# citibeth/icebin

Measured on AMD Instinct MI355X. Metric: regridded cells/sec (AvI, g5, 64 fields/GPU), higher is better.
Workload: dtype f64

## Files before the change

icebin_amd/_capi.py:

```python
import ctypes as C
import os

import numpy as np

_HERE = os.path.dirname(os.path.abspath(__file__))
LIB_PATH = os.environ.get("ICEBIN_HIP_LIB") or os.path.join(_HERE, "lib", "libicebin_hip.so")

IBH_OK, IBH_EINVAL, IBH_ENODEVICE, IBH_EHIP, IBH_ERANGE, IBH_ENOTIMPL, IBH_ENOKEY = 0, -1, -2, -3, -4, -5, -6


class IcebinHipError(RuntimeError):

    def __init__(self, code, msg):
        super().__init__(msg)
        self.code = code


class RegridderDesc(C.Structure):
    _fields_ = [
        ("nX", C.c_int64), ("ex_indices", C.c_void_p), ("ex_area", C.c_void_p), ("nI", C.c_int64),
        ("nA", C.c_int64), ("nA_dense", C.c_int32), ("A_to_sparse", C.c_void_p),
        ("A_native_area", C.c_void_p), ("A_proj_area", C.c_void_p),
        ("nhc", C.c_int32), ("hcdefs", C.c_void_p), ("hc_stride_A", C.c_int64), ("hc_stride_HC", C.c_int64),
        ("interp_style", C.c_int32), ("I_centroid_xy", C.c_void_p),
# ... 51 lines not shown
                                              C.c_void_p, C.POINTER(C.c_void_p)]),
    "ibh_regrid_matrices_matrix_batch": (C.c_int, [C.c_void_p, C.c_int32, C.c_void_p, C.c_void_p, C.c_void_p, C.c_void_p,
                                                  C.c_void_p, C.c_void_p, C.c_void_p]),
    "ibh_regrid_matrices_matrix": (C.c_int, [C.c_void_p, C.c_char_p, C.POINTER(C.c_void_p)]),
    "ibh_weighted_from_coo": (C.c_int, [C.c_int32, C.c_int32, C.c_int64, C.c_void_p, C.c_void_p, C.c_void_p,
                                       C.c_void_p, C.c_void_p, C.c_int, C.c_int, C.POINTER(C.c_void_p)]),
    "ibh_weighted_from_csr": (C.c_int, [C.c_int32, C.c_int32, C.c_void_p, C.c_void_p, C.c_void_p, C.c_void_p,
                                       C.c_void_p, C.c_int, C.c_int, C.POINTER(C.c_void_p)]),
    "ibh_e1ve0_compute": (C.c_int, [C.c_int32, C.c_void_p, C.c_void_p, C.c_int64, C.POINTER(C.c_void_p)]),
    "ibh_weighted_make_I2vX": (C.c_int, [C.c_void_p, C.c_void_p, C.c_double, C.c_void_p, C.c_int64, C.c_void_p,
                                        C.POINTER(C.c_void_p)]),
    "ibh_weighted_destroy": (C.c_int, [C.c_void_p]),
    "ibh_weighted_shape": (C.c_int, [C.c_void_p, C.POINTER(C.c_int32), C.POINTER(C.c_int32), C.POINTER(C.c_int64)]),
    "ibh_weighted_flags": (C.c_int, [C.c_void_p, C.POINTER(C.c_int), C.POINTER(C.c_int)]),
    "ibh_weighted_dim": (C.c_int, [C.c_void_p, C.c_int, C.POINTER(C.c_int64), C.POINTER(C.c_int32)]),
    "ibh_weighted_dim_to_sparse": (C.c_int, [C.c_void_p, C.c_int, C.c_void_p]),
    "ibh_weighted_get_wM": (C.c_int, [C.c_void_p, C.c_void_p]),
    "ibh_weighted_get_Mw": (C.c_int, [C.c_void_p, C.c_void_p]),
    "ibh_weighted_get_coo": (C.c_int, [C.c_void_p, C.c_void_p, C.c_void_p, C.c_void_p]),
    "ibh_weighted_get_csr": (C.c_int, [C.c_void_p, C.c_void_p, C.c_void_p, C.c_void_p]),
    "ibh_weighted_apply_host": (C.c_int, [C.c_void_p, C.c_void_p, C.c_int32, C.c_int64, C.c_void_p, C.c_int64,
                                         C.c_double, C.c_int]),
    "ibh_weighted_apply_device": (C.c_int, [C.c_void_p, C.c_void_p, C.c_int32, C.c_int64, C.c_void_p, C.c_int64,
                                           C.c_double, C.c_int, C.c_void_p]),
    "ibh_weighted_apply_many_device": (C.c_int, [C.c_void_p, C.c_int32, C.c_void_p, C.c_int32, C.c_int64, C.c_void_p,
                                                C.c_int64, C.c_double, C.c_int, C.c_void_p]),
    "ibh_weighted_matvec_device": (C.c_int, [C.c_void_p, C.c_void_p, C.c_int32, C.c_int64, C.c_void_p, C.c_int64, C.c_int,
                                            C.c_void_p]),
    "ibh_coo_matvec": (C.c_int, [C.c_void_p, C.c_void_p, C.c_int, C.c_int64, C.c_int64, C.c_int64, C.c_void_p, C.c_void_p,
                                C.c_void_p]),
    "ibh_weighted_reserve": (C.c_int, [C.c_void_p, C.c_int32]),
    "ibh_weighted_prepare": (C.c_int, [C.c_void_p, C.c_int32, C.c_int32]),
    "ibh_weighted_pair_prepare": (C.c_int, [C.c_void_p, C.c_void_p, C.c_int32]),
    "ibh_weighted_apply_chain_device": (C.c_int, [C.c_void_p, C.c_void_p, C.c_void_p, C.c_void_p, C.c_int32, C.c_int64, C.c_void_p, C.c_int64,
                                               C.c_void_p, C.c_int64, C.c_void_p, C.c_int64, C.c_double, C.c_void_p]),
    "ibh_weighted_apply_pair_device": (C.c_int, [C.c_void_p, C.c_void_p, C.c_void_p, C.c_int32, C.c_int64, C.c_void_p, C.c_int64,
                                               C.c_void_p, C.c_int64, C.c_double, C.c_void_p]),
    "ibh_comm_unique_id": (C.c_int, [C.c_char_p]),
    "ibh_comm_create": (C.c_int, [C.c_int, C.c_int, C.c_char_p, C.POINTER(C.c_void_p)]),
    "ibh_comm_create_custom": (C.c_int, [C.c_int, C.c_int, C.c_void_p, C.c_void_p, C.POINTER(C.c_void_p)]),
    "ibh_comm_destroy": (C.c_int, [C.c_void_p]),
    "ibh_comm_info": (C.c_int, [C.c_void_p, C.POINTER(C.c_int), C.POINTER(C.c_int)]),
    "ibh_comm_wait": (C.c_int, [C.c_void_p, C.c_void_p]),
    "ibh_comm_set_custom_gatherv": (C.c_int, [C.c_void_p, C.c_void_p]),
    "ibh_comm_set_stream": (C.c_int, [C.c_void_p, C.c_void_p]),
    "ibh_comm_set_option": (C.c_int, [C.c_void_p, C.c_char_p, C.c_int]),
    "ibh_regrid_matrices_matrix_d_sharded": (C.c_int, [C.c_void_p, C.c_void_p, C.c_char_p, C.c_void_p, C.c_void_p, C.c_int, C.c_int,
                                                       C.POINTER(C.c_void_p)]),
    "ibh_weighted_apply_many_sharded_device": (C.c_int, [C.c_void_p, C.c_void_p, C.c_int32, C.c_void_p, C.c_int32, C.c_int64, C.c_void_p,
                                                        C.c_int64, C.c_double, C.c_void_p]),
    "ibh_weighted_apply_sharded_device": (C.c_int, [C.c_void_p, C.c_void_p, C.c_void_p, C.c_int32, C.c_int64, C.c_void_p, C.c_int64,
                                                   C.c_double, C.c_int32, C.c_void_p]),
    "ibh_regrid_matrices_matrix_d_sharded_sigma": (C.c_int, [C.c_void_p, C.c_void_p, C.c_char_p, C.c_void_p, C.c_void_p, C.c_int, C.c_int,
                                                             C.c_void_p, C.POINTER(C.c_void_p)]),
    "ibh_weighted_apply_many_sharded_conserve_device": (C.c_int, [C.c_void_p, C.c_void_p, C.c_int32, C.c_void_p, C.c_int32, C.c_int64,
                                                                 C.c_void_p, C.c_int64, C.c_double, C.c_int, C.c_void_p]),
    "ibh_weighted_apply_sharded_conserve_device": (C.c_int, [C.c_void_p, C.c_void_p, C.c_void_p, C.c_int32, C.c_int64, C.c_void_p,
                                                            C.c_int64, C.c_double, C.c_int, C.c_int32, C.c_void_p]),
    "ibh_weighted_apply_transformed_device": (C.c_int, [C.c_void_p, C.c_void_p, C.c_int32, C.c_int64, C.c_void_p,
                                                       C.c_void_p, C.c_int32, C.c_void_p, C.c_int64, C.c_double,
                                                       C.c_void_p]),
    "ibh_weighted_apply_weight_host": (C.c_int, [C.c_void_p, C.c_int, C.c_void_p, C.c_int32, C.c_int64, C.c_void_p]),
    "ibh_weighted_device_view_get": (C.c_int, [C.c_void_p, C.POINTER(DeviceView)]),
    "ibh_weighted_set_kernel": (C.c_int, [C.c_void_p, C.c_char_p]),
    "ibh_weighted_last_kernel": (C.c_int, [C.c_void_p, C.c_char_p, C.c_int]),
    "ibh_event_create": (C.c_int, [C.POINTER(C.c_void_p)]),
# ... 95 lines not shown
```

icebin_amd/csrc/capi.hip:

```cpp
#include <algorithm>
#include <cmath>
#include <map>
#include <memory>
#include <mutex>

#include "assemble.h"
#include "common.h"
#include "prims.h"

namespace ibh {

static thread_local std::string g_last_error;
void set_last_error(const char *msg) { g_last_error = msg ? msg : ""; }
void fail(int code, const char *fmt, ...) {
    char buf[1024];
    va_list ap;
    va_start(ap, fmt);
    vsnprintf(buf, sizeof(buf), fmt, ap);
    va_end(ap);
    throw Error(code, buf);
}

namespace {
struct Pool {
// ... 521 lines not shown
        if (val) w->val.download(val, (size_t)w->nnz);
    });
}

int ibh_weighted_apply_device(const ibh_weighted *w, const double *dA, int32_t nvar, int64_t lda, double *dB,
                              int64_t ldb, double fill, int force_conservation, void *stream) {
    return guarded([&] {
        check_weighted_device(w);
        IBH_CHECK(nvar >= 0 && (nvar == 0 || (dA && dB)), "bad arguments");
        spmm_launch(w, dA, nvar, lda, dB, ldb, fill, force_conservation, static_cast<hipStream_t>(stream));
    });
}
int ibh_weighted_apply_many_device(const ibh_weighted *w, int32_t nbatch, const double *const *dA, int32_t nvar,
                                   int64_t lda, double *const *dB, int64_t ldb, double fill, int force_conservation,
                                   void *stream) {
    return guarded([&] {
        check_weighted_device(w);
        IBH_CHECK(nbatch >= 0 && nvar >= 0 && (nbatch == 0 || nvar == 0 || (dA && dB)), "bad arguments");
        spmm_launch_many(w, nbatch, dA, nvar, lda, dB, ldb, fill, force_conservation, static_cast<hipStream_t>(stream));
    });
}
int ibh_weighted_reserve(const ibh_weighted *w, int32_t nvar) {
    return guarded([&] {
        check_weighted_device(w);
        IBH_CHECK(nvar >= 0, "bad arguments");
        weighted_reserve(w, nvar);
    });
}
int ibh_weighted_prepare(const ibh_weighted *w, int32_t nvar, int32_t nbatch) {
    return guarded([&] {
        check_weighted_device(w);
        IBH_CHECK(nvar >= 0 && nbatch >= 0, "bad arguments");
        weighted_prepare(w, nvar, nbatch);
    });
}
int ibh_weighted_pair_prepare(const ibh_weighted *first, const ibh_weighted *second, int32_t nvar) {
    return guarded([&] {
        check_weighted_device(first);
        check_weighted_device(second);
        IBH_CHECK(nvar >= 0, "bad arguments");
        weighted_pair_prepare(first, second, nvar);
    });
}
int ibh_weighted_apply_pair_device(const ibh_weighted *first, const ibh_weighted *second, const double *dA, int32_t nvar, int64_t lda,
                                   double *dB1, int64_t ldb1, double *dB2, int64_t ldb2, double fill, void *stream) {
    return guarded([&] {
        check_weighted_device(first);
        check_weighted_device(second);
        IBH_CHECK(nvar >= 0 && (nvar == 0 || (dA && dB1 && dB2)), "bad arguments");
        spmm_launch_pair(first, second, dA, nvar, lda, dB1, ldb1, dB2, ldb2, fill, static_cast<hipStream_t>(stream));
    });
}
int ibh_weighted_apply_chain_device(const ibh_weighted *first, const ibh_weighted *second, const ibh_weighted *third, const double *dA, int32_t nvar,
                                    int64_t lda, double *dB1, int64_t ldb1, double *dB2, int64_t ldb2, double *dB3, int64_t ldb3, double fill,
                                    void *stream) {
    return guarded([&] {
        check_weighted_device(first);
        check_weighted_device(second);
        check_weighted_device(third);
        IBH_CHECK(nvar >= 0 && (nvar == 0 || (dA && dB1 && dB2 && dB3)), "bad arguments");
        IBH_CHECK(nvar == 0 || ldb3 >= third->nrow, "chain apply: leading dimension %ld smaller than %d rows", (long)ldb3, third->nrow);
        spmm_launch_chain(first, second, third, dA, nvar, lda, dB1, ldb1, dB2, ldb2, dB3, ldb3, fill, static_cast<hipStream_t>(stream));
    });
}
int ibh_weighted_apply_host(const ibh_weighted *w, const double *A_b, int32_t nvar, int64_t lda, double *B_b,
                            int64_t ldb, double fill, int force_conservation) {
// ... 275 lines not shown
```

icebin_amd/csrc/common.h:

```cpp
#pragma once
#include <atomic>
#include <mutex>
#include <hip/hip_runtime.h>

#include <cstdarg>
#include <cstdint>
#include <cstdio>
#include <cstring>
#include <new>
#include <stdexcept>
#include <string>
#include <unordered_map>
#include <vector>

#include "../../include/icebin_hip.h"

namespace ibh {

struct Error : std::exception {
    int code;
    std::string msg;
    Error(int c, std::string m) : code(c), msg(std::move(m)) {}
    const char *what() const noexcept override { return msg.c_str(); }
};
// ... 192 lines not shown
    mutable int64_t band_n = 0;
    mutable ibh::DevBuf<int32_t> band_ptr, band_col, band_rb1;
    mutable ibh::DevBuf<double> band_v0, band_v1;
    int band_eligible = 0;
    int64_t band_sA = 0, band_sHC = 0;
    mutable int band_tried = 0;
    mutable int64_t napply = 0;
    mutable ibh::DevBuf<double> band_part;
    mutable int sweep_tried = 0;
    mutable int32_t sweep_ntask = 0, sweep_nblk = 0, sweep_nprow = 0, sweep_nslot = 0;
    mutable int32_t sweep_tb = 0, sweep_nitems = 0, sweep_ident = 0;
    mutable ibh::DevBuf<int32_t> sweep_task_p0, sweep_task_ns, sweep_col;
    mutable ibh::DevBuf<uint32_t> sweep_meta;
    mutable ibh::DevBuf<double> sweep_v0, sweep_v1;
    mutable ibh::DevBuf<int32_t> sweep_comb_ptr, sweep_comb_p;
    mutable ibh::DevBuf<double> sweep_part;
    mutable int grp_tried = 0;
    mutable const ibh_weighted *pair_second = nullptr;
    mutable uint64_t pair_uid = 0;
    mutable ibh::DevBuf<double> pair_w;
    mutable ibh::DevBuf<uint32_t> pair_mask;
    mutable ibh::DevBuf<int32_t> pair_row;
    mutable int32_t grp_n = 0, grp_nslot = 0, grp_nitems = 0;
    mutable ibh::DevBuf<int32_t> grp_ptr, grp_ns, grp_slotrow, grp_col;
    mutable ibh::DevBuf<uint32_t> grp_meta;
    mutable ibh::DevBuf<double> grp_v0, grp_v1;
    mutable int32_t gt_ntile = 0, gt_seg = 0;
    mutable ibh::DevBuf<int32_t> gt_ptr, gt_col;
    mutable ibh::DevBuf<uint16_t> gt_ek, gt_eptr;
    mutable ibh::DevBuf<double> gt_ev;
    mutable bool have_rowsum1 = false;
    mutable ibh::DevBuf<int32_t> rowperm;
    mutable bool have_rowperm = false;
    ~ibh_weighted() {
        for (int k = 0; k < 2; ++k)
            if (owns[k]) delete dims[k];
    }
};

struct ibh_exgrid {
    int64_t nX = 0;
    ibh::DevBuf<int32_t> indices;
    ibh::DevBuf<double> overlaps;
};

namespace ibh {
int comm_world(const ibh_comm *c);
int comm_rank(const ibh_comm *c);
void comm_exchange_blocks(ibh_comm *c, double *base, int64_t count, int64_t stride, hipStream_t st);
void comm_gatherv(ibh_comm *c, int n, void *const *bases, const int64_t *const *offs, hipStream_t st);
void spmm_launch(const ibh_weighted *w, const double *dA, int nvar, int64_t lda, double *dB, int64_t ldb,
                 double fill, int force_conservation, hipStream_t stream);
void spmm_launch_many(const ibh_weighted *w, int nbatch, const double *const *dA, int nvar, int64_t lda,
                      double *const *dB, int64_t ldb, double fill, int force_conservation, hipStream_t stream);
void weighted_reserve(const ibh_weighted *w, int nvar);
void weighted_prepare(const ibh_weighted *w, int nvar, int nbatch);
void weighted_pair_prepare(const ibh_weighted *first, const ibh_weighted *second, int nvar);
void spmm_launch_pair(const ibh_weighted *first, const ibh_weighted *second, const double *dA, int nvar, int64_t lda, double *dB1,
                      int64_t ldb1, double *dB2, int64_t ldb2, double fill, hipStream_t stream);
void spmm_launch_chain(const ibh_weighted *first, const ibh_weighted *second, const ibh_weighted *third, const double *dA, int nvar, int64_t lda,
                       double *dB1, int64_t ldb1, double *dB2, int64_t ldb2, double *dB3, int64_t ldb3, double fill, hipStream_t stream);
void build_bands_from_csr(const ibh_weighted *w, hipStream_t st);
bool build_sweep_from_csr(const ibh_weighted *w, hipStream_t st);
bool build_groups_from_csr(const ibh_weighted *w, hipStream_t st);
void matvec_legacy_launch(const ibh_weighted *w, const double *dx, int nvar, int64_t ldx, double *dy, int64_t ldy,
                          int ignore_nan, hipStream_t stream);
void spmm_transformed_launch(const ibh_weighted *w, const double *dA, int nvar_in, int64_t lda, const double *T,
                              const double *b, int nvar_out, double *dB, int64_t ldb, double fill, hipStream_t stream);
void weight_dot_launch(const double *dw, int n, const double *dA, int nvar, int64_t lda, double *dout, double *part,
                       hipStream_t stream);
size_t weight_dot_scratch(int n, int nvar);
void set_launch_events(hipEvent_t start, hipEvent_t stop);
int get_tuning(const char *key, int dflt);
void set_tuning(const char *key, int value);
}
```

icebin_amd/csrc/spmm.hip:

```cpp
#include "common.h"
#include "sweep_kernel.inl"
#include <hip/hip_ext.h>
#include <mutex>

namespace ibh {

namespace {
struct Tuning {
    std::mutex mu;
    std::unordered_map<std::string, int> map;
};
Tuning &tuning() { static Tuning *t = new Tuning; return *t; }
}
static thread_local const ibh_weighted *tl_handle = nullptr;
struct HandleScope {
    const ibh_weighted *prev;
    explicit HandleScope(const ibh_weighted *w) : prev(tl_handle) { tl_handle = w; }
    ~HandleScope() { tl_handle = prev; }
};
int get_tuning(const char *key, int dflt) {
    if (tl_handle && !tl_handle->opts.empty()) {
        auto it = tl_handle->opts.find(key);
        if (it != tl_handle->opts.end()) return it->second;
    }
// ... 304 lines not shown
        const int n = min(SEG, end - seg);
        int cc[ST];
        double vv[ST];
#pragma unroll
        for (int i = 0; i < ST; ++i) {
            const int k = min((int)threadIdx.x + i * T, n - 1);
            cc[i] = colind[seg + k];
            vv[i] = vals[seg + k];
        }
        if (seg != beg) __syncthreads();
#pragma unroll
        for (int i = 0; i < ST; ++i) {
            const int k = threadIdx.x + i * T;
            if (k < n) { s_col[k] = cc[i]; s_val[k] = vv[i]; }
        }
        __syncthreads();
        double x[U];
#pragma unroll
        for (int u = 0; u < U; ++u) {
            const int k = lane + 64 * u;
            x[u] = xload(rs, s_col[k < n ? k : n - 1] << 3);
        }
        __builtin_amdgcn_sched_barrier(0);
#pragma unroll
        for (int u = 0; u < U; ++u) {
            const int k = lane + 64 * u;
            const bool ok = k < n;
            const double v = s_val[ok ? k : n - 1];
            acc = ok ? fma(v, x[u], acc) : acc;
        }
    }
    acc = wave_sum(acc);
    if (lane == 0 && fw < nf) Y[(long)fw * ldy + r] = wM[r] == 0.0 ? fill : acc;
}

struct GroupView {
    const int *ptr, *ns, *slotrow, *col;
    const unsigned *meta;
    const double *v0, *v1;
    int ngrp, nslot;
};
constexpr unsigned RG_HAS0 = 1u << 16, RG_HAS1 = 1u << 17;
struct PairView {
    const double *w;
    const unsigned *mask;
    const int *row;
    const double *wM2;
    double *Y2;
    long ldy2;
};
template <int NW, int U, int TW, bool PAIR = false>
__global__ __launch_bounds__(NW * 64) void spmm_rowgroup_kernel(const GroupView gv, const BatchPtrs bp, long ldx, int ncol, long ldy, int nf,
                                                               int nfc, int xcd_mode, const double *__restrict__ wM, double fill,
                                                               const PairView pv = PairView{})
{
    constexpr int T = NW * 64, SEG = U * 64, ST = SEG / T;
    static_assert(SEG % T == 0, "segment is a multiple of the workgroup");
    extern __shared__ double rg_lds[];
    double *s_v0 = rg_lds, *s_v1 = rg_lds + SEG;
    int *s_col = reinterpret_cast<int *>(rg_lds + 2 * SEG);
    unsigned *s_meta = reinterpret_cast<unsigned *>(s_col + SEG);
    double *s_tab = rg_lds + 3 * SEG;
    int g, fc;
    if (!block_to_task(blockIdx.x, gv.ngrp, nfc, xcd_mode, g, fc)) return;
    const int lane = threadIdx.x & 63;
    const int wave = __builtin_amdgcn_readfirstlane(threadIdx.x >> 6);
// ... 606 lines not shown
        hipExtLaunchKernelGGL((spmm_rowblock_kernel<FPW, WK, U, NW>), grid, dim3(NW * 64), 0, stream, ev0, ev1, 0,  \
                              w->rowptr.p, w->colind.p, w->val.p, bp, nbatch, qi, lda, w->ncol, ldb, w->nrow, nvar, nfc, xcd_mode, w->wM.p, fill, \
                              (const double *)nullptr, (double *)nullptr, (const int *)rowperm, 0l);     \
    } while (0)
    if (unroll == 1) IBH_RB(1);
    else if (unroll == 2) IBH_RB(2);
    else if (unroll == 8) IBH_RB(8);
    else if (unroll > 8 && FPW == 1 && WK == 1) {
        if constexpr (FPW == 1 && WK == 1 && NW == 8) {
            if (unroll <= 12) IBH_RB(12); else if (unroll <= 14) IBH_RB(14); else IBH_RB(16);
        } else IBH_RB(8);
    }
    else IBH_RB(4);
#undef IBH_RB
    IBH_HIP(hipGetLastError());
}

template <int NW, int U>
static void launch_rowone(const ibh_weighted *w, const double *X, double *Y, int nvar, long lda, long ldb, double fill, hipStream_t stream)
{
    const int nfc = ceil_div(nvar, NW);
    int xcd_mode;
    const long nb = rowblock_grid(w->nrow, nfc, xcd_mode);
    IBH_CHECK(nb < (1l << 31), "spmm grid too large (%ld blocks)", nb);
    IBH_CHECK((long)w->ncol * 8 < (1l << 31), "ncol too large for 32-bit buffer offsets");
    hipEvent_t ev0 = g_ev_start, ev1 = g_ev_stop;
    g_ev_start = g_ev_stop = nullptr;
    snprintf(w->last_sig, sizeof(w->last_sig), "spmm_rowone_kernel<%d, %d>", NW, U);
    hipExtLaunchKernelGGL((spmm_rowone_kernel<NW, U>), dim3((unsigned)nb), dim3(NW * 64), 0, stream, ev0, ev1, 0, w->rowptr.p, w->colind.p,
                          w->val.p, X, Y, lda, w->ncol, ldb, w->nrow, nvar, nfc, xcd_mode, w->wM.p, fill);
    IBH_HIP(hipGetLastError());
}

template <int NW, int U, int TW>
static void launch_rowgroup(const ibh_weighted *w, const BatchPtrs &bp, int nbatch, int nvar, long lda, long ldb, double fill, hipStream_t stream,
                            const PairView *pair = nullptr)
{
    const int nfc = ceil_div(nvar, NW);
    int xcd_mode;
    const long nb = rowblock_grid(w->grp_n, nfc, xcd_mode);
    IBH_CHECK(nb < (1l << 31), "spmm grid too large (%ld blocks)", nb);
    IBH_CHECK((long)w->ncol * 8 < (1l << 31), "ncol too large for 32-bit buffer offsets");
    GroupView gv{w->grp_ptr.p, w->grp_ns.p, w->grp_slotrow.p, w->grp_col.p, w->grp_meta.p, w->grp_v0.p, w->grp_v1.p, w->grp_n, w->grp_nslot};
    const size_t lds = (size_t)(3 * U * 64 + NW * w->grp_nslot * TW) * sizeof(double);
    hipEvent_t ev0 = g_ev_start, ev1 = g_ev_stop;
    g_ev_start = g_ev_stop = nullptr;
    if (lds > 64 * 1024) {
        static std::mutex mu;
        static bool raised[64] = {};
        std::lock_guard<std::mutex> lk(mu);
        if (!raised[w->device & 63]) {
            IBH_HIP(hipFuncSetAttribute(reinterpret_cast<const void *>(spmm_rowgroup_kernel<NW, U, TW>), hipFuncAttributeMaxDynamicSharedMemorySize, 160 * 1024));
            raised[w->device & 63] = true;
        }
    }
    snprintf(w->last_sig, sizeof(w->last_sig), "spmm_rowgroup_kernel<%d, %d, %d, %s>", NW, U, TW, pair ? "true" : "false");
    if (pair) {
        IBH_CHECK(lds <= 64 * 1024 && nbatch == 1, "fused pair apply: %zu bytes of LDS / %d batches not supported", lds, nbatch);
        hipExtLaunchKernelGGL((spmm_rowgroup_kernel<NW, U, TW, true>), dim3((unsigned)nb, 1u), dim3(NW * 64), lds, stream, ev0, ev1, 0, gv, bp,
                              lda, w->ncol, ldb, nvar, nfc, xcd_mode, w->wM.p, fill, *pair);
    } else
        hipExtLaunchKernelGGL((spmm_rowgroup_kernel<NW, U, TW>), dim3((unsigned)nb, (unsigned)nbatch), dim3(NW * 64), lds, stream, ev0, ev1, 0, gv, bp,
                              lda, w->ncol, ldb, nvar, nfc, xcd_mode, w->wM.p, fill, PairView{});
    IBH_HIP(hipGetLastError());
}

// ... 273 lines not shown
        try { build_bands_from_csr(w, stream); }
        catch (const Error &) { (void)hipGetLastError(); drop_bands(w); }
    }
}

static void size_scratch(const ibh_weighted *w, int nvar, int nbatch) {
    if (w->band_n > 0) grow_scratch(w->band_part, band_part_count(w, nvar, nbatch), nullptr, "band");
    if (w->sweep_ntask > 0) grow_scratch(w->sweep_part, sweep_part_count(w, nvar, nbatch), nullptr, "column-sweep");
    if (pick_kernel(w, nvar, nbatch) == KERNEL_SHORTROW || pick_kernel(w, nvar, 1) == KERNEL_SHORTROW || w->kernel_override == KERNEL_AUTO) {
        for (int nb : {1, nbatch}) {
            const ShortrowPlan p = shortrow_plan(w, nvar, nb);
            const int qmax = std::max(1, get_tuning("shortrow_many", w->nrow >= (1 << 19) ? 1 : IBH_MAX_BATCH));
            if (p.use_xt && (pick_kernel(w, nvar, nb) == KERNEL_SHORTROW || w->kernel_override == KERNEL_SHORTROW))
                grow_scratch(w->xt, (size_t)w->ncol * (size_t)p.ldt * (size_t)std::min(qmax, nb), nullptr, "transposed-input");
        }
    }
    grow_scratch(w->consv, 2 * (size_t)nvar + weight_dot_scratch(std::max(w->nrow, w->ncol), nvar), nullptr, "conservation");
    grow_scratch(w->scratch, (size_t)nvar * (size_t)std::min(w->nrow, w->ncol), nullptr, "transform");
    ensure_rowsum1(w, nullptr);
    if (get_tuning("rowblock_lpt", 0)) (void)ensure_rowperm(w, nullptr);
}

void weighted_reserve(const ibh_weighted *w, int nvar) {
    HandleScope hs_(w);
    if (nvar <= 0) return;
    size_scratch(w, nvar, 1);
}

void weighted_prepare(const ibh_weighted *w, int nvar, int nbatch) {
    HandleScope hs_(w);
    if (nvar <= 0 || nbatch <= 0 || w->nrow == 0) return;
    const int nb = std::min(nbatch, IBH_MAX_BATCH);
    build_structures(w, nvar, nb, true, nullptr);
    size_scratch(w, nvar, nb);
    IBH_HIP(hipStreamSynchronize(nullptr));
}

void weighted_pair_prepare(const ibh_weighted *first, const ibh_weighted *second, int nvar) {
    HandleScope hs_(first);
    IBH_CHECK(first && second && first != second, "pair: two different matrices expected");
    IBH_CHECK(first->device == second->device, "pair: matrices live on different devices");
    IBH_CHECK(second->ncol == first->nrow || second->dims[1], "pair: the second matrix's columns are not the first one's rows");
    IBH_CHECK(second->nnz <= (1 << 22), "pair: the second matrix is too large (%ld entries) to be paired on the host", (long)second->nnz);
    first->pair_second = nullptr;
    if (first->grp_n == 0) {
        const ApplyKernel keep = first->kernel_override;
        const_cast<ibh_weighted *>(first)->kernel_override = KERNEL_ROWGROUP;
        try { weighted_prepare(first, nvar > 0 ? nvar : 16, 1); } catch (...) { const_cast<ibh_weighted *>(first)->kernel_override = keep; throw; }
        const_cast<ibh_weighted *>(first)->kernel_override = keep;
    }
    if (first->grp_n == 0) fail(IBH_ENOTIMPL, "pair: the first matrix has no row groups (not an elevation-class-row matrix, or its structure was declined)");
    const int ngrp = first->grp_n;
    std::vector<int32_t> slotrow((size_t)ngrp * IBH_GSLOTS), gns((size_t)ngrp), rp2((size_t)second->nrow + 1), ci2((size_t)second->nnz);
    std::vector<double> v2((size_t)second->nnz);
    IBH_HIP(hipMemcpy(slotrow.data(), first->grp_slotrow.p, slotrow.size() * sizeof(int32_t), hipMemcpyDeviceToHost));
    IBH_HIP(hipMemcpy(gns.data(), first->grp_ns.p, gns.size() * sizeof(int32_t), hipMemcpyDeviceToHost));
    IBH_HIP(hipMemcpy(rp2.data(), second->rowptr.p, rp2.size() * sizeof(int32_t), hipMemcpyDeviceToHost));
    if (second->nnz) {
        IBH_HIP(hipMemcpy(ci2.data(), second->colind.p, ci2.size() * sizeof(int32_t), hipMemcpyDeviceToHost));
        IBH_HIP(hipMemcpy(v2.data(), second->val.p, v2.size() * sizeof(double), hipMemcpyDeviceToHost));
    }
    std::vector<int32_t> where_g((size_t)first->nrow, -1), where_s((size_t)first->nrow, -1);
    for (int g = 0; g < ngrp; ++g)
        for (int sl = 0; sl < gns[(size_t)g]; ++sl) {
            const int r = slotrow[(size_t)g * IBH_GSLOTS + sl];
            IBH_CHECK(r >= 0 && r < first->nrow, "pair: corrupt group table");
// ... 81 lines not shown
{
    if (kernel == KERNEL_ROWDUAL && g_ev_start && g_ev_stop) {
        hipEvent_t ev0 = g_ev_start, ev1 = g_ev_stop;
        g_ev_start = g_ev_stop = nullptr;
        IBH_HIP(hipEventRecord(ev0, stream));
        launch_one_impl(w, kernel, bp, nbatch, nvar, lda, ldb, fill, stream);
        IBH_HIP(hipEventRecord(ev1, stream));
        return;
    }
    launch_one_impl(w, kernel, bp, nbatch, nvar, lda, ldb, fill, stream);
}
static void launch_one_impl(const ibh_weighted *w, ApplyKernel kernel, const BatchPtrs &bp, int nbatch, int nvar, int64_t lda,
                            int64_t ldb, double fill, hipStream_t stream)
{
    if (kernel == KERNEL_ROWGROUP) {
        const int u = get_tuning("rowgroup_unroll", 8), nw = get_tuning("rowgroup_waves", nvar >= 32 ? 8 : 4);
        const int tw = get_tuning("rowgroup_tw", w->nnz < (1 << 20) ? 32 : 64);
#define IBH_RG(N, UU, TT) launch_rowgroup<N, UU, TT>(w, bp, nbatch, nvar, (long)lda, (long)ldb, fill, stream)
        if (use_grouptile(w, nvar)) {
            launch_grouptile_any(w, bp, nbatch, nvar, (long)lda, (long)ldb, fill, stream);
        } else if (tw == 32) { if (nw == 8) { if (u <= 8) IBH_RG(8, 8, 32); else IBH_RG(8, 16, 32); } else { if (u <= 4) IBH_RG(4, 4, 32); else IBH_RG(4, 8, 32); } }
        else if (nw == 8) { if (u <= 8) IBH_RG(8, 8, 64); else IBH_RG(8, 16, 64); }
        else { if (u <= 4) IBH_RG(4, 4, 64); else if (u <= 8) IBH_RG(4, 8, 64); else IBH_RG(4, 16, 64); }
#undef IBH_RG
    } else if (kernel == KERNEL_COLSWEEP) {
        launch_sweep(w, bp, nbatch, nvar, (long)lda, (long)ldb, fill, stream);
    } else if (kernel == KERNEL_ROWDUAL) {
        const long pairs = (long)w->nrow * nvar;
        const int fpw = get_tuning("rowdual_fpw", pairs >= 4 * 8192 ? 4 : pairs >= 2 * 8192 ? 2 : 1);
        if (fpw >= 4) launch_rowdual<4>(w, bp, nbatch, nvar, (long)lda, (long)ldb, fill, stream);
        else if (fpw == 2) launch_rowdual<2>(w, bp, nbatch, nvar, (long)lda, (long)ldb, fill, stream);
        else launch_rowdual<1>(w, bp, nbatch, nvar, (long)lda, (long)ldb, fill, stream);
    } else if (kernel == KERNEL_ROWBLOCK) {
        int fpw = get_tuning(nbatch > 1 ? "rowblock_many_fpw" : "rowblock_fpw", 0), wk = get_tuning("rowblock_wk", 0);
        if (fpw == 0 || wk == 0) {
            const long pairs = (long)w->nrow * nvar;
            if (nvar >= 16 && pairs >= 4 * 8192) { fpw = 4; wk = 1; }
            else if (nvar >= 8 && pairs >= 2 * 8192) { fpw = 2; wk = 1; }
            else if (nvar >= 4) { fpw = 1; wk = 1; }
            else if (nvar >= 2) { fpw = 1; wk = 2; }
            else { fpw = 1; wk = 4; }
        }
        const double mean_len = w->nrow ? (double)w->nnz / (double)w->nrow : 0.0;
        const int rowone = get_tuning("rowone", nbatch == 1 && wk == 1 && nvar >= 32 && mean_len >= 192.0 && mean_len <= 1024.0 ? 1 : 0);
        if (rowone && nbatch == 1 && wk == 1) {
            int u = get_tuning("rowone_unroll", mean_len > 768.0 ? 16 : 14), nw = get_tuning("rowone_waves", 8);
            const double *X1 = bp.x[0];
            double *Y1 = bp.y[0];
#define IBH_R1(N, UU) launch_rowone<N, UU>(w, X1, Y1, nvar, (long)lda, (long)ldb, fill, stream)
            if (nw == 4) { if (u <= 8) IBH_R1(4, 8); else if (u <= 12) IBH_R1(4, 12); else IBH_R1(4, 14); }
            else { if (u <= 8) IBH_R1(8, 8); else if (u <= 12) IBH_R1(8, 12); else if (u <= 14) IBH_R1(8, 14); else IBH_R1(8, 16); }
#undef IBH_R1
            return;
        }
        const int nw = get_tuning("rowblock_waves", nbatch >= 8 && fpw == 1 && wk == 1 ? 8 : 4);
#define IBH_L(F, K, N) launch_rowblock<F, K, N>(w, bp, nbatch, nvar, (long)lda, (long)ldb, fill, stream)
        if (nw == 8 && wk == 1) {
            if (fpw == 1) IBH_L(1, 1, 8); else if (fpw == 2) IBH_L(2, 1, 8); else IBH_L(4, 1, 8);
        } else if (fpw == 4 && wk == 1) IBH_L(4, 1, 4);
        else if (fpw == 8 && wk == 1) IBH_L(8, 1, 4);
        else if (fpw == 2 && wk == 1) IBH_L(2, 1, 4);
        else if (fpw == 1 && wk == 1) IBH_L(1, 1, 4);
        else if (fpw == 4 && wk == 2) IBH_L(4, 2, 4);
        else if (fpw == 2 && wk == 2) IBH_L(2, 2, 4);
        else if (fpw == 1 && wk == 2) IBH_L(1, 2, 4);
        else if (fpw == 2 && wk == 4) IBH_L(2, 4, 4);
// ... 32 lines not shown
                hipExtLaunchKernelGGL(transpose_fields_kernel, dim3((unsigned)ceil_div(w->ncol, 64), (unsigned)(p.ldt / 16), (unsigned)nq), dim3(256), 0, stream,
                                      e_first, nullptr, 0, bq, (long)lda, nvar, w->ncol, w->xt.p, p.ldt, xt_stride);
                e_first = nullptr;
                xld = p.ldt;
            }
#define IBH_SR4(NT, GG, RA, XTT)                                                                                        \
    snprintf(w->last_sig, sizeof(w->last_sig), "%s", "spmm_shortrow_kernel<" #NT ", " #GG ", " #RA ", " #XTT ">");      \
    hipExtLaunchKernelGGL((spmm_shortrow_kernel<NT, GG, RA, XTT>), grid, dim3(SR_THREADS), 0, stream, e_first, e_last, 0,  \
                          w->rowptr.p, w->colind.p, w->val.p, bq, (const double *)w->xt.p, xt_stride, xld, (long)ldb,       \
                          w->nrow, nvar, fper, w->wM.p, fill)
#define IBH_SR(NT, GG)                                                                                          \
    do {                                                                                                        \
        if (realign) { if (p.use_xt) { IBH_SR4(NT, GG, true, true); } else { IBH_SR4(NT, GG, true, false); } }  \
        else { if (p.use_xt) { IBH_SR4(NT, GG, false, true); } else { IBH_SR4(NT, GG, false, false); } }        \
    } while (0)
            const bool nt = get_tuning("shortrow_nt", 1) != 0;
            if (g >= 16) { if (nt) IBH_SR(true, 16); else IBH_SR(false, 16); }
            else if (g >= 8) { if (nt) IBH_SR(true, 8); else IBH_SR(false, 8); }
            else { if (nt) IBH_SR(true, 4); else IBH_SR(false, 4); }
#undef IBH_SR4
#undef IBH_SR
        }
        IBH_HIP(hipGetLastError());
    }
}

void spmm_launch_many(const ibh_weighted *w, int nbatch, const double *const *dA, int nvar, int64_t lda,
                      double *const *dB, int64_t ldb, double fill, int force_conservation, hipStream_t stream)
{
    HandleScope hs_(w);
    if (nvar <= 0 || w->nrow == 0 || nbatch <= 0) return;
    IBH_CHECK(lda >= w->ncol && ldb >= w->nrow, "apply: leading dimensions (%ld, %ld) smaller than (%d, %d)",
              (long)lda, (long)ldb, w->ncol, w->nrow);
    if (get_tuning("lazy_structures", 1)) build_structures(w, nvar, std::min(nbatch, IBH_MAX_BATCH), w->napply >= 1, stream, (long)w->napply);
    ++w->napply;
    ApplyKernel kernel = pick_kernel(w, nvar, nbatch);
    if (kernel == KERNEL_COLSWEEP && ((uint64_t)16 * (uint64_t)lda * 8 + (uint64_t)w->ncol * 8 >= (1ull << 32)))
        kernel = w->band_n > 0 ? KERNEL_ROWDUAL : KERNEL_ROWBLOCK;
    w->last_kernel = kernel;
    w->last_sig[0] = 0;
    const bool correct = !w->conservative && force_conservation;
    if (correct) grow_scratch(w->consv, 2 * (size_t)nvar + weight_dot_scratch(std::max(w->nrow, w->ncol), nvar), stream, "conservation");
    for (int b0 = 0; b0 < nbatch; b0 += IBH_MAX_BATCH) {
        const int nb = std::min(IBH_MAX_BATCH, nbatch - b0);
        BatchPtrs bp{};
        for (int q = 0; q < nb; ++q) {
            IBH_CHECK(dA[b0 + q] && dB[b0 + q], "apply: null field pointer in batch %d", b0 + q);
            bp.x[q] = dA[b0 + q]; bp.y[q] = dB[b0 + q];
        }
        launch_one(w, kernel, bp, nb, nvar, lda, ldb, fill, stream);
        if (correct) {
            for (int q = 0; q < nb; ++q) {
                double *T = w->consv.p;
                weight_dot_launch(w->Mw.p, w->ncol, bp.x[q], nvar, lda, T, T + 2 * nvar, stream);
                weight_dot_launch(w->wM.p, w->nrow, bp.y[q], nvar, ldb, T + nvar, T + 2 * nvar, stream);
                dim3 grid((unsigned)ceil_div(w->nrow, 256), (unsigned)nvar);
                hipLaunchKernelGGL(conserve_scale_kernel, grid, dim3(256), 0, stream, bp.y[q], (long)ldb, w->nrow, w->wM.p,
                                   T, T + nvar);
            }
            IBH_HIP(hipGetLastError());
        }
    }
}

void spmm_launch(const ibh_weighted *w, const double *dA, int nvar, int64_t lda, double *dB, int64_t ldb,
                 double fill, int force_conservation, hipStream_t stream)
{
// ... 128 lines not shown
```

include/icebin_hip.h:

```cpp
#ifndef ICEBIN_HIP_H
#define ICEBIN_HIP_H

#include <stdint.h>

#ifdef __cplusplus
extern "C" {
#endif

#define IBH_OK          0
#define IBH_EINVAL     -1
#define IBH_ENODEVICE  -2
#define IBH_EHIP       -3
#define IBH_ERANGE     -4
#define IBH_ENOTIMPL   -5
#define IBH_ENOKEY     -6

const char *ibh_last_error(void);
int ibh_version(void);
int ibh_device_count(int *count);
int ibh_set_device(int device);

typedef struct ibh_sparse_set ibh_sparse_set;
int ibh_sparse_set_create(int64_t sparse_extent, ibh_sparse_set **out);
int ibh_sparse_set_create_identity(int64_t n, ibh_sparse_set **out);
// ... 112 lines not shown
                          const double *wM , const double *Mw ,
                          int conservative, int scaled, ibh_weighted **out);
int ibh_weighted_from_csr(int32_t nrow, int32_t ncol, const int32_t *rowptr,
                          const int32_t *colind, const double *val,
                          const double *wM, const double *Mw,
                          int conservative, int scaled, ibh_weighted **out);
int ibh_weighted_destroy(ibh_weighted *w);

int ibh_e1ve0_compute(int32_t nsheets, const ibh_weighted *const *XuE1s, const ibh_weighted *const *XuE0s,
                      int64_t nE, ibh_weighted **out);

int ibh_weighted_make_I2vX(const ibh_weighted *IvX, const ibh_hntr *hIvI2, double eq_rad, const uint8_t *includeI, int64_t nincl,
                           ibh_sparse_set *dimI2, ibh_weighted **out);

int ibh_weighted_shape(const ibh_weighted *w, int32_t *nrow_d, int32_t *ncol_d, int64_t *nnz);
int ibh_weighted_flags(const ibh_weighted *w, int *conservative, int *scaled);
int ibh_weighted_dim(const ibh_weighted *w, int k, int64_t *sparse_extent, int32_t *dense_extent);
int ibh_weighted_dim_to_sparse(const ibh_weighted *w, int k, int64_t *out );
int ibh_weighted_get_wM(const ibh_weighted *w, double *out );
int ibh_weighted_get_Mw(const ibh_weighted *w, double *out );
int ibh_weighted_get_coo(const ibh_weighted *w, int32_t *row, int32_t *col, double *val);
int ibh_weighted_get_csr(const ibh_weighted *w, int32_t *rowptr, int32_t *colind, double *val);

int ibh_weighted_apply_host(const ibh_weighted *w, const double *A_b, int32_t nvar, int64_t lda,
                            double *B_b, int64_t ldb, double fill, int force_conservation);
int ibh_weighted_apply_device(const ibh_weighted *w, const double *dA_b, int32_t nvar, int64_t lda,
                              double *dB_b, int64_t ldb, double fill, int force_conservation,
                              void *stream);
#define IBH_MAX_BATCH 32
int ibh_weighted_apply_many_device(const ibh_weighted *w, int32_t nbatch, const double *const *dA_b, int32_t nvar,
                                   int64_t lda, double *const *dB_b, int64_t ldb, double fill,
                                   int force_conservation, void *stream);
int ibh_weighted_prepare(const ibh_weighted *w, int32_t nvar, int32_t nbatch);

int ibh_weighted_pair_prepare(const ibh_weighted *first, const ibh_weighted *second, int32_t nvar);
int ibh_weighted_apply_pair_device(const ibh_weighted *first, const ibh_weighted *second, const double *dA_b, int32_t nvar, int64_t lda,
                                   double *dB1_b, int64_t ldb1, double *dB2_b, int64_t ldb2, double fill, void *stream);
int ibh_weighted_apply_chain_device(const ibh_weighted *first, const ibh_weighted *second, const ibh_weighted *third, const double *dA_b,
                                    int32_t nvar, int64_t lda, double *dB1_b, int64_t ldb1, double *dB2_b, int64_t ldb2, double *dB3_b,
                                    int64_t ldb3, double fill, void *stream);
int ibh_weighted_reserve(const ibh_weighted *w, int32_t nvar);
int ibh_weighted_apply_transformed_device(const ibh_weighted *w, const double *dA_b, int32_t nvar_in, int64_t lda,
                                          const double *T, const double *b, int32_t nvar_out,
                                          double *dB_b, int64_t ldb, double fill, void *stream);
int ibh_weighted_matvec_device(const ibh_weighted *w, const double *dxx, int32_t nvar, int64_t ldx,
                               double *dyy, int64_t ldy, int ignore_nan, void *stream);
int ibh_coo_matvec(double *yy , const double *xx , int ignore_nan,
                   int64_t nrow, int64_t ncol, int64_t nnz, const int32_t *row, const int32_t *col,
                   const double *data);
int ibh_weighted_apply_weight_host(const ibh_weighted *w, int dim, const double *A_b,
                                   int32_t nvar, int64_t lda, double *out );

#define IBH_UNIQUE_ID_BYTES 128
typedef struct ibh_comm ibh_comm;
typedef int (*ibh_exchange_fn)(void *user, double *d_base, int64_t count, int64_t stride, int world, int rank, void *stream);
int ibh_comm_unique_id(char id[IBH_UNIQUE_ID_BYTES]);
int ibh_comm_create(int world, int rank, const char id[IBH_UNIQUE_ID_BYTES], ibh_comm **out);
int ibh_comm_create_custom(int world, int rank, ibh_exchange_fn fn, void *user, ibh_comm **out);
typedef int (*ibh_gatherv_fn)(void *user, void *d_base, const int64_t *offsets, int world, int rank, void *stream);
int ibh_comm_set_custom_gatherv(ibh_comm *c, ibh_gatherv_fn fn);
int ibh_comm_set_stream(ibh_comm *c, void *stream);
int ibh_comm_set_option(ibh_comm *c, const char *key, int value);
int ibh_comm_destroy(ibh_comm *c);
int ibh_comm_info(const ibh_comm *c, int *world, int *rank);
int ibh_weighted_apply_sharded_device(const ibh_weighted *w, ibh_comm *c, const double *dA_local, int32_t nvar_local,
                                      int64_t lda, double *dB_all, int64_t ldb, double fill, int32_t block_fields,
// ... 48 lines not shown
```

Baseline: 668.1 billion.

## Add row-run SpMM kernel loading contiguous column runs via buffer-to-LDS

Adds a new batched row-block SpMM kernel for matrices whose rows consist mostly of one contiguous column run. It precomputes, on the host, the longest consecutive-column run per row. The kernel fetches that run with 16-byte buffer loads straight into LDS instead of doing per-element gathers through colind. Remaining entries still use indexed loads. The kernel is enabled only when runs cover at least 75% of nonzeros, no row exceeds the kernel's maximum length, nbatch > 1 and nvar >= 8. The cost is a one-time device-to-host copy and host scan, plus heavy LDS use per block, which may limit occupancy.

```diff
diff --git a/icebin_amd/_capi.py b/icebin_amd/_capi.py
--- a/icebin_amd/_capi.py
+++ b/icebin_amd/_capi.py
@@ -107,6 +107,7 @@
     "ibh_weighted_reserve": (C.c_int, [C.c_void_p, C.c_int32]),
     "ibh_weighted_prepare": (C.c_int, [C.c_void_p, C.c_int32, C.c_int32]),
     "ibh_weighted_pair_prepare": (C.c_int, [C.c_void_p, C.c_void_p, C.c_int32]),
+    "ibh_csr_row_runs": (C.c_int, [C.c_int32, C.c_void_p, C.c_void_p, C.c_void_p, C.c_void_p, C.c_void_p, C.POINTER(C.c_int64)]),
     "ibh_weighted_apply_chain_device": (C.c_int, [C.c_void_p, C.c_void_p, C.c_void_p, C.c_void_p, C.c_int32, C.c_int64, C.c_void_p, C.c_int64,
                                                C.c_void_p, C.c_int64, C.c_void_p, C.c_int64, C.c_double, C.c_void_p]),
     "ibh_weighted_apply_pair_device": (C.c_int, [C.c_void_p, C.c_void_p, C.c_void_p, C.c_int32, C.c_int64, C.c_void_p, C.c_int64,
diff --git a/icebin_amd/csrc/capi.hip b/icebin_amd/csrc/capi.hip
--- a/icebin_amd/csrc/capi.hip
+++ b/icebin_amd/csrc/capi.hip
@@ -577,6 +577,12 @@
         check_weighted_device(w);
         IBH_CHECK(nvar >= 0 && nbatch >= 0, "bad arguments");
         weighted_prepare(w, nvar, nbatch);
+    });
+}
+int ibh_csr_row_runs(int32_t nrow, const int32_t *rowptr, const int32_t *colind, int32_t *k0, int32_t *len, int32_t *c0, int64_t *covered) {
+    return guarded([&] {
+        IBH_CHECK(nrow >= 0 && rowptr && k0 && len && c0 && covered && (nrow == 0 || rowptr[nrow] == 0 || colind), "bad arguments");
+        *covered = row_runs_host(nrow, rowptr, colind, k0, len, c0);
     });
 }
 int ibh_weighted_pair_prepare(const ibh_weighted *first, const ibh_weighted *second, int32_t nvar) {
diff --git a/icebin_amd/csrc/common.h b/icebin_amd/csrc/common.h
--- a/icebin_amd/csrc/common.h
+++ b/icebin_amd/csrc/common.h
@@ -248,6 +248,9 @@
     mutable bool have_rowsum1 = false;
     mutable ibh::DevBuf<int32_t> rowperm;
     mutable bool have_rowperm = false;
+    mutable int run_tried = 0;
+    mutable bool run_ok = false;
+    mutable ibh::DevBuf<int32_t> run_k0, run_len, run_c0;
     ~ibh_weighted() {
         for (int k = 0; k < 2; ++k)
             if (owns[k]) delete dims[k];
@@ -271,6 +274,7 @@
                       double *const *dB, int64_t ldb, double fill, int force_conservation, hipStream_t stream);
 void weighted_reserve(const ibh_weighted *w, int nvar);
 void weighted_prepare(const ibh_weighted *w, int nvar, int nbatch);
+int64_t row_runs_host(int nrow, const int32_t *rowptr, const int32_t *colind, int32_t *k0, int32_t *len, int32_t *c0);
 void weighted_pair_prepare(const ibh_weighted *first, const ibh_weighted *second, int nvar);
 void spmm_launch_pair(const ibh_weighted *first, const ibh_weighted *second, const double *dA, int nvar, int64_t lda, double *dB1,
                       int64_t ldb1, double *dB2, int64_t ldb2, double fill, hipStream_t stream);
diff --git a/icebin_amd/csrc/spmm.hip b/icebin_amd/csrc/spmm.hip
--- a/icebin_amd/csrc/spmm.hip
+++ b/icebin_amd/csrc/spmm.hip
@@ -360,6 +360,82 @@
     }
     acc = wave_sum(acc);
     if (lane == 0 && fw < nf) Y[(long)fw * ldy + r] = wM[r] == 0.0 ? fill : acc;
+}
+
+constexpr int RR_U = 14, RR_NW = 8, RR_MAX = RR_U * 64;
+__global__ __launch_bounds__(RR_NW * 64, 4) void spmm_rowrun_kernel(
+    const int *__restrict__ rowptr, const int *__restrict__ colind, const double *__restrict__ vals,
+    const int *__restrict__ run_k0, const int *__restrict__ run_len, const int *__restrict__ run_c0,
+    const BatchPtrs bp, int nbatch, int qi, long ldx, int ncol, long ldy, int nrow, int nf, int nfc,
+    int xcd_mode, const double *__restrict__ wM, double fill, int nt)
+{
+    constexpr int T = RR_NW * 64, ST = (RR_MAX + T - 1) / T;
+    __shared__ int s_col[RR_MAX];
+    __shared__ double s_val[RR_MAX];
+    __shared__ __attribute__((aligned(16))) double s_run[RR_NW][RR_MAX];
+    int r, fc;
+    if (!block_to_task(blockIdx.x, nrow, nfc, xcd_mode, r, fc)) return;
+    const int lane = threadIdx.x & 63;
+    const int wave = __builtin_amdgcn_readfirstlane(threadIdx.x >> 6);
+    const int fw = fc * RR_NW + wave;
+    const int f = fw < nf ? fw : nf - 1;
+    const int q0 = blockIdx.y * qi, q1 = min(nbatch, q0 + qi);
+    const int beg = rowptr[r], n = rowptr[r + 1] - beg;
+    const int k0 = run_k0[r], len = run_len[r], c0 = run_c0[r];
+    const bool dead = wM[r] == 0.0;
+#pragma unroll
+    for (int i = 0; i < ST; ++i) {
+        const int k = threadIdx.x + i * T;
+        if (k < n) {
+            s_val[k] = vals[beg + k];
+            if ((unsigned)(k - k0) >= (unsigned)len) s_col[k] = colind[beg + k];
+        }
+    }
+    __syncthreads();
+    double *buf = s_run[wave];
+    for (int q = q0; q < q1; ++q) {
+        const double *plane = bp.x[q] + (long)f * ldx;
+        const __amdgpu_buffer_rsrc_t rs = __builtin_amdgcn_make_buffer_rsrc((void *)plane, 0, ncol * 8, 0x00020000);
+        const int h = (int)((reinterpret_cast<uintptr_t>(plane + c0) >> 3) & 1);
+        const int m = len > h ? (len - h) & ~1 : 0;
+        const int kr = k0 + h;
+        for (int c = 0; c < m; c += 128) {
+            const int e = c + 2 * lane;
+            auto *lds = (__attribute__((address_space(3))) void *)(buf + c);
+            if (e < m) {
+                if (nt) __builtin_amdgcn_raw_ptr_buffer_load_lds(rs, lds, 16, (c0 + h + e) * 8, 0, 0, 2);
+                else __builtin_amdgcn_raw_ptr_buffer_load_lds(rs, lds, 16, (c0 + h + e) * 8, 0, 0, 0);
+            }
+        }
+        double x[RR_U];
+#pragma unroll
+        for (int u = 0; u < RR_U; ++u) {
+            const int k = lane + 64 * u;
+            x[u] = 0.0;
+            if (k < n && (unsigned)(k - kr) >= (unsigned)m) {
+                const int col = (unsigned)(k - k0) < (unsigned)len ? c0 + (k - k0) : s_col[k];
+                x[u] = xload(rs, col << 3);
+            }
+        }
+        __builtin_amdgcn_s_waitcnt(0x0f70);
+#pragma unroll
+        for (int u = 0; u < RR_U; ++u) {
+            const int k = lane + 64 * u;
+            if ((unsigned)(k - kr) < (unsigned)m) x[u] = buf[k - kr];
+        }
+        double acc = 0.0;
+        if (n > 0) {
+#pragma unroll
+            for (int u = 0; u < RR_U; ++u) {
+                const int k = lane + 64 * u;
+                const bool ok = k < n;
+                const double v = s_val[ok ? k : n - 1];
+                acc = ok ? fma(v, x[u], acc) : acc;
+            }
+        }
+        acc = wave_sum(acc);
+        if (lane == 0 && fw < nf) bp.y[q][(long)fw * ldy + r] = dead ? fill : acc;
+    }
 }
 
 struct GroupView {
@@ -1032,6 +1108,76 @@
     IBH_HIP(hipGetLastError());
 }
 
+int64_t row_runs_host(int nrow, const int32_t *rowptr, const int32_t *colind, int32_t *k0, int32_t *len, int32_t *c0) {
+    int64_t covered = 0;
+    for (int r = 0; r < nrow; ++r) {
+        const int beg = rowptr[r], end = rowptr[r + 1];
+        int bk = 0, bl = 0;
+        for (int k = beg; k < end;) {
+            int e = k + 1;
+            while (e < end && colind[e] == colind[e - 1] + 1) ++e;
+            if (e - k > bl) { bk = k - beg; bl = e - k; }
+            k = e;
+        }
+        k0[r] = bk; len[r] = bl; c0[r] = bl ? colind[beg + bk] : 0;
+        covered += bl;
+    }
+    return covered;
+}
+static void ensure_row_runs(const ibh_weighted *w, hipStream_t stream) {
+    if (w->run_tried) return;
+    hipStreamCaptureStatus cs = hipStreamCaptureStatusNone;
+    if (stream) IBH_HIP(hipStreamIsCapturing(stream, &cs));
+    if (cs != hipStreamCaptureStatusNone) return;
+    w->run_tried = 1;
+    if (w->nrow < 1 || w->nnz < 1) return;
+    std::vector<int32_t> rp((size_t)w->nrow + 1);
+    IBH_HIP(hipMemcpyAsync(rp.data(), w->rowptr.p, rp.size() * sizeof(int32_t), hipMemcpyDeviceToHost, stream));
+    IBH_HIP(hipStreamSynchronize(stream));
+    for (int r = 0; r < w->nrow; ++r)
+        if (rp[(size_t)r + 1] - rp[(size_t)r] > RR_MAX) return;
+    std::vector<int32_t> ci((size_t)w->nnz), k0((size_t)w->nrow), len((size_t)w->nrow), c0((size_t)w->nrow);
+    IBH_HIP(hipMemcpyAsync(ci.data(), w->colind.p, ci.size() * sizeof(int32_t), hipMemcpyDeviceToHost, stream));
+    IBH_HIP(hipStreamSynchronize(stream));
+    const int64_t covered = row_runs_host(w->nrow, rp.data(), ci.data(), k0.data(), len.data(), c0.data());
+    if (4 * covered < 3 * w->nnz) return;
+    w->run_k0.upload(k0.data(), k0.size(), stream);
+    w->run_len.upload(len.data(), len.size(), stream);
+    w->run_c0.upload(c0.data(), c0.size(), stream);
+    IBH_HIP(hipStreamSynchronize(stream));
+    w->run_ok = true;
+}
+
+static void launch_rowrun(const ibh_weighted *w, const BatchPtrs &bp, int nbatch, int nvar, long lda, long ldb, double fill,
+                          hipStream_t stream)
+{
+    const int nfc = ceil_div(nvar, RR_NW);
+    int xcd_mode;
+    const long nb = rowblock_grid(w->nrow, nfc, xcd_mode);
+    IBH_CHECK(nb < (1l << 31), "spmm grid too large (%ld blocks)", nb);
+    IBH_CHECK((long)w->ncol * 8 < (1l << 31), "ncol too large for 32-bit buffer offsets");
+    int qi = get_tuning("rowrun_qi", get_tuning("rowblock_many_qi", 0));
+    if (qi <= 0) qi = nbatch >= 4 ? 2 : 1;
+    if (qi > nbatch) qi = nbatch;
+    const dim3 grid((unsigned)nb, (unsigned)ceil_div(nbatch, qi));
+    const int nt = get_tuning("rowrun_nt", 0) != 0;
+    hipEvent_t ev0 = g_ev_start, ev1 = g_ev_stop;
+    g_ev_start = g_ev_stop = nullptr;
+    snprintf(w->last_sig, sizeof(w->last_sig), "spmm_rowrun_kernel");
+    hipExtLaunchKernelGGL(spmm_rowrun_kernel, grid, dim3(RR_NW * 64), 0, stream, ev0, ev1, 0, w->rowptr.p, w->colind.p, w->val.p,
+                          w->run_k0.p, w->run_len.p, w->run_c0.p, bp, nbatch, qi, lda, w->ncol, ldb, w->nrow, nvar, nfc, xcd_mode,
+                          w->wM.p, fill, nt);
+    IBH_HIP(hipGetLastError());
+}
+static bool use_rowrun(const ibh_weighted *w, int nvar, int nbatch) {
+    if (nbatch <= 1 || !w->run_ok) return false;
+    const int force = get_tuning("rowrun", -1);
+    if (force >= 0) return force != 0;
+    for (const char *key : {"rowblock_many_fpw", "rowblock_fpw", "rowblock_wk", "rowblock_waves", "rowblock_unroll", "rowblock_lpt"})
+        if (get_tuning(key, INT32_MIN) != INT32_MIN) return false;
+    return nvar >= 8;
+}
+
 template <int NW, int U, int TW>
 static void launch_rowgroup(const ibh_weighted *w, const BatchPtrs &bp, int nbatch, int nvar, long lda, long ldb, double fill, hipStream_t stream,
                             const PairView *pair = nullptr)
@@ -1371,6 +1517,7 @@
     if (nvar <= 0 || nbatch <= 0 || w->nrow == 0) return;
     const int nb = std::min(nbatch, IBH_MAX_BATCH);
     build_structures(w, nvar, nb, true, nullptr);
+    if (nb > 1 && pick_kernel(w, nvar, nb) == KERNEL_ROWBLOCK) ensure_row_runs(w, nullptr);
     size_scratch(w, nvar, nb);
     IBH_HIP(hipStreamSynchronize(nullptr));
 }
@@ -1518,6 +1665,10 @@
         else if (fpw == 2) launch_rowdual<2>(w, bp, nbatch, nvar, (long)lda, (long)ldb, fill, stream);
         else launch_rowdual<1>(w, bp, nbatch, nvar, (long)lda, (long)ldb, fill, stream);
     } else if (kernel == KERNEL_ROWBLOCK) {
+        if (use_rowrun(w, nvar, nbatch)) {
+            launch_rowrun(w, bp, nbatch, nvar, (long)lda, (long)ldb, fill, stream);
+            return;
+        }
         int fpw = get_tuning(nbatch > 1 ? "rowblock_many_fpw" : "rowblock_fpw", 0), wk = get_tuning("rowblock_wk", 0);
         if (fpw == 0 || wk == 0) {
             const long pairs = (long)w->nrow * nvar;
@@ -1616,7 +1767,10 @@
     if (nvar <= 0 || w->nrow == 0 || nbatch <= 0) return;
     IBH_CHECK(lda >= w->ncol && ldb >= w->nrow, "apply: leading dimensions (%ld, %ld) smaller than (%d, %d)",
               (long)lda, (long)ldb, w->ncol, w->nrow);
-    if (get_tuning("lazy_structures", 1)) build_structures(w, nvar, std::min(nbatch, IBH_MAX_BATCH), w->napply >= 1, stream, (long)w->napply);
+    if (get_tuning("lazy_structures", 1)) {
+        build_structures(w, nvar, std::min(nbatch, IBH_MAX_BATCH), w->napply >= 1, stream, (long)w->napply);
+        if (nbatch > 1 && pick_kernel(w, nvar, nbatch) == KERNEL_ROWBLOCK) ensure_row_runs(w, stream);
+    }
     ++w->napply;
     ApplyKernel kernel = pick_kernel(w, nvar, nbatch);
     if (kernel == KERNEL_COLSWEEP && ((uint64_t)16 * (uint64_t)lda * 8 + (uint64_t)w->ncol * 8 >= (1ull << 32)))
diff --git a/include/icebin_hip.h b/include/icebin_hip.h
--- a/include/icebin_hip.h
+++ b/include/icebin_hip.h
@@ -168,6 +168,8 @@
                                    int64_t lda, double *const *dB_b, int64_t ldb, double fill,
                                    int force_conservation, void *stream);
 int ibh_weighted_prepare(const ibh_weighted *w, int32_t nvar, int32_t nbatch);
+int ibh_csr_row_runs(int32_t nrow, const int32_t *rowptr, const int32_t *colind, int32_t *k0, int32_t *len, int32_t *c0,
+                     int64_t *covered);
 
 int ibh_weighted_pair_prepare(const ibh_weighted *first, const ibh_weighted *second, int32_t nvar);
 int ibh_weighted_apply_pair_device(const ibh_weighted *first, const ibh_weighted *second, const double *dA_b, int32_t nvar, int64_t lda,
```

New measurement: 533.6 billion, median of 2. 0.799x the previous value.
